# sadPororo/AD-YOLO

Hardware: AMD Instinct MI355X
Metric: train-step audio-sec/s (4ch, se-resnet34+adyolo) (higher is better)
Workload: dtype f32; 1 GPU; se-resnet34 + adyolo loss, synthetic 4ch 24kHz 60s clips, bs=64 per GPU, 12 classes, features+fwd+loss+bwd+allreduce+Adam; global_batch=64, parallelism=dp1

## Files before the change

### ad-yolo_amd/_lib.py

```python
import ctypes
import os

_HERE = os.path.dirname(os.path.abspath(__file__))
LIB_PATH = os.environ.get("ADYOLO_LIB") or os.path.join(_HERE, "libadyolo_hip.so")

P = ctypes.c_void_p
I = ctypes.c_int
L = ctypes.c_long
F = ctypes.c_float
U64 = ctypes.c_uint64

SIGNATURES = {
    "adyolo_abi_version": (I, []),
    "adyolo_last_error": (ctypes.c_char_p, []),
    "adyolo_feat_stft_mel": (I, [P] * 8 + [I, I] + [P] * 4 + [I, I, I, P]),
    "adyolo_feat_finish": (I, [P] * 4 + [I, I, I, P]),
    "adyolo_feat_gcc_phat": (I, [P] * 6 + [I, I, I, I, P]),
    "adyolo_nchw_to_nhwc8": (I, [P, P, I, I, I, I, P]),
    "adyolo_pack_w3x3": (I, [P, P, P, I, I, I, P]),
    "adyolo_conv3x3_tiles": (I, [I] * 3),
    "adyolo_conv3x3_fwd": (I, [P] * 13 + [I] * 7 + [P]),
    "adyolo_wino_pack_w": (I, [P, P, P, I, I, I, P]),
    "adyolo_wino_pack_many": (I, [P, I, I, I, P]),
    "adyolo_wino_tiles": (I, [I] * 3),
    "adyolo_wino_fwd": (I, [P] * 13 + [I] * 7 + [P]),
    "adyolo_wino4_pack_w": (I, [P, P, P, I, I, I, P]),
    "adyolo_wino4_pack_many": (I, [P, I, I, I, P]),
    "adyolo_wino4_tiles": (I, [I] * 3),
    "adyolo_wino4_fwd": (I, [P] * 13 + [I] * 7 + [P]),
    "adyolo_wino4_fwd_form": (I, [I] * 3),
    "adyolo_wino4_last_form": (I, []),
    "adyolo_set_switches": (I, [I]),
    "adyolo_wino4_wgrad_slabs": (I, [I] * 5),
    "adyolo_wino4_wgrad": (I, [P] * 7 + [I] * 6 + [P]),
    "adyolo_wino_wgrad_slabs": (I, [I] * 5),
    "adyolo_wino_wgrad": (I, [P] * 7 + [I] * 6 + [P]),
    "adyolo_conv3x3_wgrad_slabs": (I, [I] * 5),
    "adyolo_conv3x3_wgrad": (I, [P] * 6 + [I] * 6 + [P]),
    "adyolo_gemm": (I, [P] * 5 + [I] * 10 + [P]),
    "adyolo_gemm_batched": (I, [P] * 3 + [I] * 10 + [L] * 6 + [F, I, P]),
    "adyolo_colsum": (I, [P, P, P, I, I, I, I, P]),
    "adyolo_bn_stats": (I, [P] * 7 + [I, I, I, F, F, P]),
    "adyolo_bn_stats_tiles": (I, [P] * 11 + [I, I, I, I, F, F, P]),
    "adyolo_bn_eval_stats": (I, [P] * 4 + [I, F, P]),
    "adyolo_bn_scale_shift": (I, [P] * 6 + [I, P]),
    "adyolo_affine_nhwc": (I, [P] * 4 + [L, I, P]),
    "adyolo_bn_bwd_reduce": (I, [P] * 7 + [L, I, P]),
    "adyolo_bn_bwd_tiles": (I, [P, P, P, P, I, I, P]),
    "adyolo_bn_bwd_apply": (I, [P] * 12 + [L, I, I, F, P]),
    "adyolo_bn_persample": (I, [P, P, P, I, I, I, P]),
    "adyolo_bn_finish": (I, [P] * 10 + [I, I, I, F, F, P]),
    "adyolo_se_fc_fwd": (I, [P] * 10 + [I, I, I, I, P]),
    "adyolo_relu_mask_words": (L, [I, I, I]),
    "adyolo_se_tail_fwd": (I, [P] * 9 + [I, I, I, P]),
    "adyolo_se_tail_fwd_pool_ok": (I, [I, I, I]),
    "adyolo_se_tail_fwd_pool": (I, [P] * 9 + [I, I, I, I, P]),
    "adyolo_se_tail_bwd_reduce": (I, [P] * 9 + [I, I, I, P]),
    "adyolo_se_tail_bwd_tiles": (I, [P, P, P, I, I, I, P]),
    "adyolo_se_fc_bwd_words": (L, [I, I]),
    "adyolo_se_fc_bwd": (I, [P] * 16 + [I, I, I, I, P]),
    "adyolo_se_tail_bwd_apply": (I, [P] * 13 + [I, I, I, F, P]),
    "adyolo_se_tail_bwd_reduce_pooled": (I, [P] * 8 + [I, I, I, I, P]),
    "adyolo_se_tail_bwd_apply_pooled": (I, [P] * 13 + [I, I, I, I, F, P]),
    "adyolo_avgpool2_fwd": (I, [P, P, I, I, I, I, P]),
    "adyolo_avgpool2_bwd": (I, [P, P, I, I, I, I, P]),
    "adyolo_add": (I, [P, P, P, L, P]),
    "adyolo_mul": (I, [P, P, P, L, P]),
    "adyolo_scale_dev": (I, [P, P, P, L, P]),
    "adyolo_sap_fwd": (I, [P] * 5 + [I, I, I, P]),
    "adyolo_sap_bwd": (I, [P] * 8 + [I, I, I, P]),
    "adyolo_gru_fwd": (I, [P] * 6 + [I, I, P]),
    "adyolo_gru_bwd": (I, [P] * 6 + [I, I, P]),
# ... 113 lines not shown
```

### ad-yolo_amd/csrc/gemm.hip

```cpp
#include "common.hpp"

namespace adyolo {

constexpr int GBM = 128, GBN = 64, GBK = 32;
#ifndef GEMM_WHATIF
#define GEMM_WHATIF 0
#endif
#ifndef GEMM_ST_NT
#define GEMM_ST_NT 0
#endif
#ifndef GEMM_PF
#define GEMM_PF 1
#endif

struct GemmBatch {
    int inner;
    long oA, iA, oB, iB, oC, iC;
    float alpha;
};

struct ConvGather {
    int Hs, Ws, Cs, Hm, Wm, KH, KW, SH, SW, PH, PW, dgrad, kreal;
};

// ... 386 lines not shown
#pragma unroll
        for (int nt = 0; nt < SN; ++nt) {
            const int nn = n0 + (wn * SN + nt) * 32 + li;
#pragma unroll
            for (int r = 0; r < 16; ++r) {
                const int m = m0 + (wm * SM + sm) * 32 + mfma_row(r, lane);
                if (m < M && nn < N && (!(GEMM_WHATIF & 1) || r == 0)) {
                    if (slab_stride) {
                        C[(size_t)z * slab_stride + (size_t)m * slab_ld + nn] = acc[sm][nt][r];
                    } else {
                        float v = acc[sm][nt][r] * bt.alpha;
                        if (bias) v += bias[nn];
                        const size_t o = (size_t)m * ldc + nn;
                        if (accumulate) v += C[o];
                        C[o] = v;
                    }
                }
            }
        }
}

__global__ void gemm_slab_reduce_kernel(const float *__restrict__ slabs, const float *__restrict__ bias,
                                        float *__restrict__ C, int M, int N, int ldc, int splits, int accumulate) {
    const size_t idx = (size_t)blockIdx.x * blockDim.x + threadIdx.x;
    const size_t total = (size_t)M * N;
    if (idx >= total) return;
    const int m = (int)(idx / N), nn = (int)(idx - (size_t)m * N);
    float s = 0.f;
    for (int z = 0; z < splits; ++z) s += slabs[(size_t)z * total + idx];
    if (bias) s += bias[nn];
    const size_t o = (size_t)m * ldc + nn;
    if (accumulate) s += C[o];
    C[o] = s;
}

__global__ __launch_bounds__(256) void colsum_partial_kernel(const float *__restrict__ A, float *__restrict__ partial,
                                                             long R, int C, int lda, long rows_per_block) {
    __shared__ float red[256];
    const int cx = threadIdx.x & 63, ry = threadIdx.x >> 6;
    const int c = blockIdx.y * 64 + cx;
    const long rbeg = (long)blockIdx.x * rows_per_block;
    const long rend = rbeg + rows_per_block < R ? rbeg + rows_per_block : R;
    float s = 0.f;
    if (c < C)
        for (long r = rbeg + ry; r < rend; r += 4) s += A[(size_t)r * lda + c];
    red[threadIdx.x] = s;
    __syncthreads();
    if (ry == 0 && c < C) partial[(size_t)blockIdx.x * C + c] = red[cx] + red[64 + cx] + red[128 + cx] + red[192 + cx];
}
__global__ __launch_bounds__(256) void colsum_final_kernel(const float *__restrict__ partial, float *__restrict__ out,
                                                           int nblk, int C, int accumulate) {
    __shared__ double red[256];
    const double s = block_colsum32(partial, nblk, (size_t)C, blockIdx.x * 32, C, red);
    const int c = blockIdx.x * 32 + (threadIdx.x & 31);
    if ((threadIdx.x >> 5) == 0 && c < C) out[c] = (accumulate ? out[c] : 0.f) + (float)s;
}

__global__ void add_kernel(const float4 *__restrict__ a, const float4 *__restrict__ b, float4 *__restrict__ y,
                           long n4) {
    for (long i = (long)blockIdx.x * blockDim.x + threadIdx.x; i < n4; i += (long)gridDim.x * blockDim.x) {
        const float4 u = a[i], v = b[i];
        y[i] = make_float4(u.x + v.x, u.y + v.y, u.z + v.z, u.w + v.w);
    }
}
__global__ void mul_kernel(const float4 *__restrict__ a, const float4 *__restrict__ b, float4 *__restrict__ y,
                           long n4) {
// ... 118 lines not shown
    } else if (mode == 1) {
        M = N * H * W, Nn = Cin, K = Kq;
        cg = ConvGather{Ho, Wo, Cout, H, W, KH, KW, SH, SW, PH, PW, 1, KH * KW * Cout};
    } else {
        M = Cout, Nn = Kp, K = N * Ho * Wo;
        cg = ConvGather{H, W, Cin, Ho, Wo, KH, KW, SH, SW, PH, PW, 0, KH * KW * Cin};
    }
    if (mode != 2 || splits < 1) splits = mode == 2 ? (splits < 1 ? 1 : splits) : 1;
    ADYOLO_REQUIRE(splits == 1 || slabs, ADYOLO_EINVAL, "conv_gemm: splits > 1 needs a slab workspace");
    const int klen = cdiv(cdiv(K, splits), GBK) * GBK;
    splits = cdiv(K, klen);
    int fastg = mode == 2 ? (gemm_fast_fetch(M, 4, K, Cout, 4, 1, 1, klen) & 1)
                          : (gemm_fast_fetch(4, Nn, K, 4, mode == 0 ? Kp : Kq, 0, 0, klen) & 2);
    if (fastg && mode != 2 && cg.Cs % GBK == 0 && (mode == 0 || (SH == 1 && SW == 1)) &&
        (long)N * cg.Hs * cg.Ws * cg.Cs + (long)(KH * cg.Ws + KW) * cg.Cs < ((long)1 << 29))
        fastg |= 4;
    dim3 grid((unsigned)cdiv(Nn, GBN), (unsigned)cdiv(M, GBM), (unsigned)splits);
    const size_t slab_stride = splits > 1 ? (size_t)M * Nn : 0;
    float *dst = splits > 1 ? slabs : out;
    if (mode == 2)
        hipLaunchKernelGGL((gemm_kernel<true, true, 2>), grid, dim3(256), 0, st, other, src, bias, dst, M, Nn, K, Cout, 0,
                           Nn, klen, slab_stride, Nn, 0, bt, cg, fastg);
    else
        hipLaunchKernelGGL((gemm_kernel<false, false, 1>), grid, dim3(256), 0, st, src, other, bias, dst, M, Nn, K, 0,
                           mode == 0 ? Kp : Kq, Nn, klen, slab_stride, Nn, 0, bt, cg, fastg);
    int rc = check_launch("conv_gemm");
    if (rc || splits == 1) return rc;
    const size_t total = (size_t)M * Nn;
    hipLaunchKernelGGL(gemm_slab_reduce_kernel, dim3(cdiv((long)total, 256)), dim3(256), 0, st, slabs, bias, out, M, Nn,
                       Nn, splits, 0);
    return check_launch("conv_gemm_reduce");
}

extern "C" int adyolo_colsum(const float *A, float *out, float *partial, int R, int C, int lda, int accumulate,
                             void *stream) {
    ADYOLO_REQUIRE(A && out && partial && R > 0 && C > 0, ADYOLO_EINVAL, "colsum: bad arguments");
    hipStream_t st = as_stream(stream);
    int nblk = cdiv(R, 64);
    if (nblk > 1024) nblk = 1024;
    const long rpb = ((long)R + nblk - 1) / nblk;
    nblk = cdiv(R, rpb);
    hipLaunchKernelGGL(colsum_partial_kernel, dim3(nblk, cdiv(C, 64)), dim3(256), 0, st, A, partial, (long)R, C, lda, rpb);
    int rc = check_launch("colsum_partial");
    if (rc) return rc;
    hipLaunchKernelGGL(colsum_final_kernel, dim3(cdiv(C, 32)), dim3(256), 0, st, partial, out, nblk, C, accumulate);
    return check_launch("colsum_final");
}

extern "C" int adyolo_add(const float *a, const float *b, float *y, long n, void *stream) {
    ADYOLO_REQUIRE(a && b && y && n > 0 && n % 4 == 0, ADYOLO_EINVAL, "add: n must be a positive multiple of 4");
    const long n4 = n / 4;
    const int grid = (int)(n4 / 256 + 1 > 4096 ? 4096 : n4 / 256 + 1);
    hipLaunchKernelGGL(add_kernel, dim3(grid), dim3(256), 0, as_stream(stream), (const float4 *)a, (const float4 *)b,
                       (float4 *)y, n4);
    return check_launch("add");
}
extern "C" int adyolo_mul(const float *a, const float *b, float *y, long n, void *stream) {
    ADYOLO_REQUIRE(a && b && y && n > 0 && n % 4 == 0, ADYOLO_EINVAL, "mul: n must be a positive multiple of 4");
    const long n4 = n / 4;
    const int grid = (int)(n4 / 256 + 1 > 4096 ? 4096 : n4 / 256 + 1);
    hipLaunchKernelGGL(mul_kernel, dim3(grid), dim3(256), 0, as_stream(stream), (const float4 *)a, (const float4 *)b,
                       (float4 *)y, n4);
    return check_launch("mul");
}
```

### ad-yolo_amd/csrc/wino4w.hip

```cpp
#include "wino4_common.hpp"

namespace adyolo {
namespace w4 {

#ifndef W4W_WHATIF
#define W4W_WHATIF 0
#endif
#ifndef W4W_LD_AUX
#define W4W_LD_AUX 0
#endif
#ifndef W4W_TIMING
#define W4W_TIMING 0
#endif

__device__ __forceinline__ void a6v(const f32x4 (&v)[4], f32x4 (&t)[6]) {
    auto fm = [](float k, f32x4 a, f32x4 b) { return pkfma4(k, a, b); };
    const f32x4 z = {0.f, 0.f, 0.f, 0.f};
    const f32x4 ea = fm(A2, v[2], v[0]), oa = fm(A3, v[3], fm(PA, v[1], z));
    const f32x4 eb = fm(B2, v[2], v[0]), ob = fm(B3, v[3], fm(PB, v[1], z));
    t[0] = v[0];
    t[1] = ea + oa;
    t[2] = fm(-1.f, oa, ea);
    t[3] = eb + ob;
    t[4] = fm(-1.f, ob, eb);
// ... 364 lines not shown
            }
            tstamp(2);
            if (NB == 2) {
                d_xform_full();
                __builtin_amdgcn_sched_barrier(0);
#pragma unroll
                for (int s = 0; s < 9; ++s) {
                    side(9 + s);
                    __builtin_amdgcn_sched_barrier(0);
                    mfma4(s, 1);
                    __builtin_amdgcn_sched_barrier(0);
                }
            }
            tstamp(3);
            tstamp(4);
#if W4W_TIMING
            ++tstep;
#endif
        };
        for (int k = 0; k < nsteps;) {
            step(std::integral_constant<int, 0>{}, k);
            if (++k >= nsteps) break;
            step(std::integral_constant<int, 4>{}, k);
            if (++k >= nsteps) break;
            step(std::integral_constant<int, 8>{}, k);
            if (++k >= nsteps) break;
            step(std::integral_constant<int, 2>{}, k);
            if (++k >= nsteps) break;
            step(std::integral_constant<int, 6>{}, k);
            ++k;
        }
    }

#pragma unroll
    for (int s = 0; s < 9; ++s) {
        const int pos = wave * 9 + s;
#pragma unroll
        for (int cb = 0; cb < NB; ++cb)
#pragma unroll
            for (int r = 0; r < 16; ++r) {
                const int m = mfma_row(r, lane);
                slabs[(((size_t)split * 36 + pos) * Cin + c0 + m) * Cout + co0 + cb * 32 + li] = acc[s][cb][r];
            }
    }
}

__global__ __launch_bounds__(256) void wino4_wgrad_reduce_kernel(const float *__restrict__ slabs, float *__restrict__ du, int nslab,
                                                                 int pairs) {
    __shared__ double red[256];
    const int p = blockIdx.y, total = 36 * pairs;
    const double s = block_colsum32(slabs, nslab, (size_t)total, p * pairs + blockIdx.x * 32, p * pairs + pairs, red);
    const int idx = blockIdx.x * 32 + (threadIdx.x & 31);
    if ((threadIdx.x >> 5) == 0 && idx < pairs) du[(size_t)p * pairs + idx] = (float)s;
}
__global__ __launch_bounds__(256) void wino4_wgrad_finish_kernel(const float *__restrict__ du, float *__restrict__ dw, int Cin,
                                                                 int Cin_real, int Cout) {
    const int pairs = Cin * Cout;
    const int idx = blockIdx.x * blockDim.x + threadIdx.x;
    if (idx >= pairs) return;
    const int co = idx % Cout, ci = idx / Cout;
    if (ci >= Cin_real) return;
    double d[6][6];
#pragma unroll
    for (int wv = 0; wv < 4; ++wv)
#pragma unroll
        for (int s = 0; s < 9; ++s) {
            const int p = wv * 9 + s;
            const int nu = s < 6 ? (wv == 0 ? 0 : wv == 1 ? 2 : wv == 2 ? 3 : 5) : (wv < 2 ? 1 : 4);
            const int xi = s < 6 ? s : (wv & 1) ? (s == 6 ? 5 : s - 4) : s - 6;
            d[xi][nu] = (double)du[(size_t)p * pairs + idx];
        }
    const double a_ = 0.75, b_ = 1.5, a2 = a_ * a_, b2 = b_ * b_;
    const double na = 2.0 * a2 * (a2 - b2), nb = 2.0 * b2 * (b2 - a2);
    const double G[6][3] = {{1.0 / (a2 * b2), 0.0, 0.0}, {1.0 / na, a_ / na, a2 / na}, {1.0 / na, -a_ / na, a2 / na},
                            {1.0 / nb, b_ / nb, b2 / nb}, {1.0 / nb, -b_ / nb, b2 / nb}, {0.0, 0.0, 1.0}};
    float *o = dw + ((size_t)co * Cin_real + ci) * 9;
#pragma unroll
    for (int ky = 0; ky < 3; ++ky)
#pragma unroll
        for (int kx = 0; kx < 3; ++kx) {
            double s_ = 0.0;
#pragma unroll
            for (int xi = 0; xi < 6; ++xi) {
                double r_ = 0.0;
#pragma unroll
                for (int nu = 0; nu < 6; ++nu) r_ += d[xi][nu] * G[nu][kx];
                s_ += G[xi][ky] * r_;
            }
            o[ky * 3 + kx] = (float)s_;
        }
}

static int wino4_wgrad_geometry(int N, int H, int W, int Cin, int Cout, int *npairs_o, int *nseg_o, int *seg_steps_o, int *nitems_o,
                                int *nblk_o) {
    const int nruns = W >= 16 ? N * (W / 16) : cdiv(N, 16 / W), npairs = (nruns + 1) / 2;
    const int nblk = (Cout / (Cout % 64 == 0 ? 64 : 32)) * (Cin / 32);
    int nsplit = 256 / nblk;
    if (nsplit < 1) nsplit = 1;
    const int steps = H / 4;
    int nseg = 1, seg_steps = steps;
    {
        long best = -1;
        const int maxseg = steps >= 16 ? steps / 8 : 1;
        for (int c = 1; c <= maxseg; ++c) {
            const int ss = (steps + c - 1) / c;
            const int ns = (steps + ss - 1) / ss;
            const long items = (long)npairs * ns;
            const int sp = nsplit < items ? nsplit : (int)items;
            const long cost = ((items + sp - 1) / sp) * (long)(ss + 2);
            if (best < 0 || cost < best) {
                best = cost;
                nseg = ns;
                seg_steps = ss;
            }
        }
    }
    const int nitems = npairs * nseg;
    if (nsplit > nitems) nsplit = nitems;
    if (npairs_o) *npairs_o = npairs;
    if (nseg_o) *nseg_o = nseg;
    if (seg_steps_o) *seg_steps_o = seg_steps;
    if (nitems_o) *nitems_o = nitems;
    if (nblk_o) *nblk_o = nblk;
    return nsplit;
}

}
}

using namespace adyolo;

#if W4W_TIMING
extern "C" int adyolo_w4w_timing_buffer(void *p) {
    return hipMemcpyToSymbol(HIP_SYMBOL(w4::g_w4w_stamps), &p, sizeof(p)) == hipSuccess ? 0 : -1;
}
#endif

extern "C" int adyolo_wino4_wgrad_slabs(int N, int H, int W, int Cin, int Cout) {
    if (N <= 0 || H <= 0 || W <= 0 || Cin <= 0 || Cout <= 0) return ADYOLO_EINVAL;
    if (Cin % 32 || Cout % 32 || (W % 16 && W != 4 && W != 8) || H % 4 || H < 8) return 0;
    if ((size_t)N * H * W * (size_t)(Cin > Cout ? Cin : Cout) * 4 >= ((size_t)1 << 31)) return 0;
    return w4::wino4_wgrad_geometry(N, H, W, Cin, Cout, nullptr, nullptr, nullptr, nullptr, nullptr);
}

extern "C" int adyolo_wino4_wgrad(const float *x, const float *dy, const float *in_scale, const float *in_shift, float *slabs,
                                  float *du, float *dw, int N, int H, int W, int Cin, int Cin_real, int Cout, void *stream) {
    ADYOLO_REQUIRE(x && dy && slabs && du && dw && N > 0 && H > 0 && W > 0, ADYOLO_EINVAL, "wino4_wgrad: bad arguments");
    ADYOLO_REQUIRE(adyolo_wino4_wgrad_slabs(N, H, W, Cin, Cout) > 0 && Cin_real > 0 && Cin_real <= Cin, ADYOLO_ENOSUP,
                   "wino4_wgrad: unsupported shape N=%d H=%d W=%d Cin=%d Cout=%d (needs Cin %% 32 == 0, Cout %% 32 == 0, W %% 16 == 0 or W = 4 | 8, "
                   "H %% 4 == 0, tensors below 2 GiB)", N, H, W, Cin, Cout);
    ADYOLO_REQUIRE((in_scale == nullptr) == (in_shift == nullptr), ADYOLO_EINVAL, "wino4_wgrad: in_scale/in_shift come together");
    ADYOLO_REQUIRE(((reinterpret_cast<size_t>(x) | reinterpret_cast<size_t>(dy) | reinterpret_cast<size_t>(in_scale) |
                     reinterpret_cast<size_t>(in_shift)) & 15) == 0, ADYOLO_ENOSUP, "wino4_wgrad: x, dy, in_scale, in_shift must be 16-byte aligned");
    hipStream_t st = as_stream(stream);
    int npairs, nseg, seg_steps, nitems, nblk;
    const int nsplit = w4::wino4_wgrad_geometry(N, H, W, Cin, Cout, &npairs, &nseg, &seg_steps, &nitems, &nblk);
    const unsigned grid = (unsigned)(nsplit * nblk);
#define ADYOLO_W4W(AFF_, NB_)                                                                                          \
    hipLaunchKernelGGL((w4::wino4_wgrad_kernel<AFF_, NB_>), dim3(grid), dim3(256), 0, st, x, dy, in_scale, in_shift, slabs, N, H, \
                       W, Cin, Cout, W >= 16 ? W / 16 : -(W / 4), npairs, nseg, seg_steps, nitems, nsplit, Cin / 32, nblk)
    if (Cout % 64 == 0) {
        if (in_scale) ADYOLO_W4W(true, 2); else ADYOLO_W4W(false, 2);
    } else {
        if (in_scale) ADYOLO_W4W(true, 1); else ADYOLO_W4W(false, 1);
    }
#undef ADYOLO_W4W
    int rc = check_launch("wino4_wgrad");
    if (rc) return rc;
    hipLaunchKernelGGL(w4::wino4_wgrad_reduce_kernel, dim3(cdiv(Cin * Cout, 32), 36), dim3(256), 0, st, slabs, du, nsplit, Cin * Cout);
    rc = check_launch("wino4_wgrad_reduce");
    if (rc) return rc;
    hipLaunchKernelGGL(w4::wino4_wgrad_finish_kernel, dim3(cdiv(Cin * Cout, 256)), dim3(256), 0, st, du, dw, Cin, Cin_real, Cout);
    return check_launch("wino4_wgrad_finish");
}
```

### ad-yolo_amd/ops.py

```python
import ctypes
import os

import numpy as np
import torch

from . import _lib

_c = _lib.call
NULL = ctypes.c_void_p(0)


def _p(t):
    if t is None:
        return NULL
    return ctypes.c_void_p(t.data_ptr())


def _stream():
    return ctypes.c_void_p(torch.cuda.current_stream().cuda_stream)


def _chk(*ts):
    for t in ts:
        if t is None:
# ... 265 lines not shown
    if isinstance(wpk, DualPack):
        wpk = wpk.pick(n, h, w, cout, addend is not None, w4_form == 2)
    form = wpk.shape[0] if wpk.dim() == 4 else 0
    if form == 36 and not w4_form:
        raise _lib.AdyoloHipError("conv3x3: a F(4x4) pack with %d output channels needs an operand combination the persistent kernel "
                                  "is built for (pack with ops.DualPack / WinoPackSet to fall back to F(2x2))" % cout)
    fn, tiles_fn, name = _CONV3X3_FORMS[form]
    _chk(x, wpk, bias, addend, None if mbits & 1 else addend_mask, None if mbits & 2 else stat_mask)
    y = _new(x, n, h, w, cout)
    stats = _new(x, 2, getattr(lib, tiles_fn)(n, h, w), cout) if want_stats else None
    sc, sh = in_affine if in_affine is not None else (None, None)
    sa, sm, si = stat_bn if stat_bn is not None else (None, None, None)
    _c(fn, _p(x), _p(wpk), _p(bias), _p(addend), _p(addend_mask),
       _p(sc), _p(sh), _p(y), _p(stats), _p(sa), _p(sm), _p(si), _p(stat_mask), n, h, w, cin, cout, int(relu), mbits,
       _stream())
    if DISPATCH_LOG is not None:
        k = (name or _W4_KERNELS[w4_form], cin, cout, epi)
        DISPATCH_LOG[k] = DISPATCH_LOG.get(k, 0) + 1
    return (y, stats) if want_stats else y


def wgrad_form(cin, cout, algo=None, shape=None):
    algo = algo or W4_THRESHOLDS["wgrad_algo"] or conv_algo()
    if algo == "winograd4" and shape is not None and cin % 32 == 0 and cout % 32 == 0:
        n, h, w = shape
        if (w % 16 == 0 or w in (4, 8)) and h % 4 == 0 and n * w // 16 * (h // 4) * cin * cout >= W4_THRESHOLDS["min_wgrad_work"] and \
                _lib.load().adyolo_wino4_wgrad_slabs(n, h, w, cin, cout) > 0:
            return "wino4_wgrad_kernel", 9.0 / 36.0
    if algo in ("winograd", "winograd4") and cin % 32 == 0 and cout % 32 == 0:
        return "wino_wgrad_kernel", 16.0 / 36.0
    return "conv3x3_wgrad_kernel", 1.0


_WGRAD_FORMS = {"wino4_wgrad_kernel": ("adyolo_wino4_wgrad", 36), "wino_wgrad_kernel": ("adyolo_wino_wgrad", 16)}


def conv3x3_wgrad(x, dy, cin_real, in_affine=None, algo=None, out=None):
    _chk(x, dy)
    n, h, w, cin = x.shape
    cout = dy.shape[3]
    sc, sh = in_affine if in_affine is not None else (None, None)
    dw = out if out is not None else _new(x, cout, cin_real, 3, 3)
    form = wgrad_form(cin, cout, algo, (n, h, w))[0]
    if DISPATCH_LOG is not None:
        k = (form, cin, cout, 1 if in_affine is not None else 0)
        DISPATCH_LOG[k] = DISPATCH_LOG.get(k, 0) + 1
    if form in _WGRAD_FORMS:
        fn, points = _WGRAD_FORMS[form]
        nslab = getattr(_lib.load(), fn + "_slabs")(n, h, w, cin, cout)
        if nslab <= 0:
            raise _lib.AdyoloHipError("%s_slabs rejected the shape" % fn)
        slabs = _new(x, nslab, points, cin, cout)
        du = _new(x, points, cin, cout)
        _c(fn, _p(x), _p(dy), _p(sc), _p(sh), _p(slabs), _p(du), _p(dw), n, h, w, cin, cin_real, cout, _stream())
        return dw
    nslab = _lib.load().adyolo_conv3x3_wgrad_slabs(n, h, w, cin, cout)
    if nslab <= 0:
        raise _lib.AdyoloHipError("conv3x3_wgrad_slabs rejected the shape")
    cinp = ((cin + 31) // 32) * 32
    slabs = _new(x, nslab, cout, 9, cinp)
    _c("adyolo_conv3x3_wgrad", _p(x), _p(dy), _p(sc), _p(sh), _p(slabs), _p(dw), n, h, w, cin, cin_real, cout, _stream())
    return dw


def gemm(a, b, m, n, k, lda, ldb, trans_a=False, trans_b=False, bias=None, out=None, ldc=None, accumulate=False,
         splits=1):
    if ldc is None:
        ldc = n
    if out is None:
        out = _new(a, m, n)
        ldc = n
    slabs = None
    if splits > 1:
        slabs = _new(a, splits, m, n)
    _c("adyolo_gemm", _p(a), _p(b), _p(bias), _p(out), _p(slabs), m, n, k, lda, ldb, ldc, int(trans_a), int(trans_b),
       splits, int(accumulate), _stream())
    return out


def wgrad_splits(m, n, k):
    tiles = ((m + 127) // 128) * ((n + 63) // 64)
    want = (512 + tiles - 1) // tiles
    return max(1, min(256, want, k // 512))


def linear(x2d, w, bias=None):
    _chk(x2d, w, bias)
    r, k = x2d.shape
    return gemm(x2d, w, r, w.shape[0], k, k, k, bias=bias)


def linear_bwd(x2d, w, dy2d, need_dx=True, out_dw=None, out_db=None, need_db=True):
    _chk(x2d, w, dy2d)
    r, k = x2d.shape
    n = w.shape[0]
    dx = gemm(dy2d, w, r, k, n, n, k, trans_b=True) if need_dx else None
    dw = gemm(dy2d, x2d, n, k, r, n, k, trans_a=True, trans_b=True, splits=wgrad_splits(n, k, r), out=out_dw)
    db = colsum(dy2d, out=out_db) if need_db else None
    return dx, dw, db


def colsum(a2d, out=None, accumulate=False):
    r, c = a2d.shape
    if out is None:
        out = _new(a2d, c)
        accumulate = False
    partial = _new(a2d, 1024, c)
    _c("adyolo_colsum", _p(a2d), _p(out), _p(partial), r, c, a2d.stride(0), int(accumulate), _stream())
    return out


def add(a, b):
    _chk(a, b)
    y = torch.empty_like(a)
    _c("adyolo_add", _p(a), _p(b), _p(y), a.numel(), _stream())
    return y


def scale_dev(a, scalar_dev):
    _chk(a, scalar_dev)
    y = torch.empty_like(a)
    _c("adyolo_scale_dev", _p(a), _p(scalar_dev), _p(y), a.numel(), _stream())
    return y


def mul(a, b):
    _chk(a, b)
    y = torch.empty_like(a)
    _c("adyolo_mul", _p(a), _p(b), _p(y), a.numel(), _stream())
# ... 975 lines not shown
```

### include/adyolo_hip.h

```cpp
#ifndef ADYOLO_HIP_H
#define ADYOLO_HIP_H

#include <stddef.h>
#include <stdint.h>

#ifdef __cplusplus
extern "C" {
#endif

#define ADYOLO_ABI_VERSION 2
#define ADYOLO_EINVAL (-1)
#define ADYOLO_ENOSUP (-2)

int         adyolo_abi_version(void);
const char *adyolo_last_error(void);

int adyolo_feat_stft_mel(const float *audio, const int64_t *clip_offset, const float *twiddle,
                         const int32_t *chunk_mel, const int32_t *chunk_start, const int32_t *chunk_len,
                         const int32_t *chunk_off, const float *mel_w, int n_chunks, int n_mel_w,
                         const float *scaler_mean, const float *scaler_rstd, float *out, float *chan_max, int B,
                         int n_samples, int layout, void *stream);
int adyolo_feat_finish(float *out, const float *chan_max, const float *scaler_mean,
                       const float *scaler_rstd, int B, int T, int layout, void *stream);

// ... 7 lines not shown
                     void *stream);
int adyolo_conv3x3_tiles(int N, int H, int W);
int adyolo_conv3x3_fwd(const float *x, const float *wpk, const float *bias, const float *addend,
                       const float *addend_mask, const float *in_scale, const float *in_shift, float *y,
                       float *stats, const float *stat_aux, const float *stat_mean, const float *stat_invstd,
                       const float *stat_mask, int N, int H, int W, int Cin, int Cout, int relu, int mask_bits, void *stream);
int adyolo_wino_pack_w(const float *w , float *u_fwd , float *u_dgrad ,
                       int Cout, int Cin_real, int Cin, void *stream);
int adyolo_wino_pack_many(const int64_t *table, int n, int max_cout, int max_cin, void *stream);
int adyolo_wino_tiles(int N, int H, int W);
int adyolo_wino_fwd(const float *x, const float *u, const float *bias, const float *addend,
                    const float *addend_mask, const float *in_scale, const float *in_shift, float *y, float *stats,
                    const float *stat_aux, const float *stat_mean, const float *stat_invstd, const float *stat_mask,
                    int N, int H, int W, int Cin, int Cout, int relu, int mask_bits, void *stream);
int adyolo_wino4_pack_w(const float *w , float *u_fwd , float *u_dgrad ,
                        int Cout, int Cin_real, int Cin, void *stream);
int adyolo_wino4_pack_many(const int64_t *table, int n, int max_cout, int max_cin, void *stream);
int adyolo_wino4_tiles(int N, int H, int W);
int adyolo_wino4_fwd(const float *x, const float *u, const float *bias, const float *addend, const float *addend_mask,
                     const float *in_scale, const float *in_shift, float *y, float *stats, const float *stat_aux,
                     const float *stat_mean, const float *stat_invstd, const float *stat_mask, int N, int H, int W, int Cin,
                     int Cout, int relu, int mask_bits, void *stream);
#define ADYOLO_W4_STATS 1
#define ADYOLO_W4_ADDEND 2
#define ADYOLO_W4_ADDEND_MASK 4
#define ADYOLO_W4_STAT_AUX 8
#define ADYOLO_W4_STAT_MASK 16
#define ADYOLO_W4_BIAS 32
int adyolo_wino4_fwd_form(int Cout, int operands, int mask_bits);
int adyolo_wino4_last_form(void);
int adyolo_set_switches(int bits);
int adyolo_wino4_wgrad_slabs(int N, int H, int W, int Cin, int Cout);
int adyolo_wino4_wgrad(const float *x, const float *dy, const float *in_scale , const float *in_shift ,
                       float *slabs, float *du , float *dw, int N, int H, int W, int Cin, int Cin_real,
                       int Cout, void *stream);
int adyolo_wino_wgrad_slabs(int N, int H, int W, int Cin, int Cout);
int adyolo_wino_wgrad(const float *x, const float *dy, const float *in_scale, const float *in_shift, float *slabs,
                      float *du, float *dw, int N, int H, int W, int Cin, int Cin_real, int Cout, void *stream);
int adyolo_conv3x3_wgrad_slabs(int N, int H, int W, int Cin, int Cout);
int adyolo_conv3x3_wgrad(const float *x, const float *dy, const float *in_scale, const float *in_shift,
                         float *slabs, float *dw, int N, int H, int W, int Cin, int Cin_real, int Cout,
                         void *stream);

int adyolo_gemm(const float *A, const float *B, const float *bias, float *C, float *slabs, int M,
                int N, int K, int lda, int ldb, int ldc, int transA, int transB, int splits,
                int accumulate, void *stream);
int adyolo_gemm_batched(const float *A, const float *B, float *C, int M, int N, int K, int lda, int ldb, int ldc,
                        int transA, int transB, int outer, int inner, long oA, long iA, long oB, long iB, long oC,
                        long iC, float alpha, int accumulate, void *stream);
int adyolo_colsum(const float *A, float *out, float *partial, int R, int C, int lda, int accumulate,
                  void *stream);

int adyolo_bn_stats(const float *x, float *ssum, float *mean, float *invstd, float *running_mean,
                    float *running_var, float *partial, int N, int HW, int C, float momentum,
                    float eps, void *stream);
int adyolo_bn_stats_tiles(const float *tile_stats, float *ssum, float *mean, float *invstd, float *running_mean,
                          float *running_var, const float *gamma, const float *beta, float *scale, float *shift,
                          float *partial, int N, int G, int HW, int C, float momentum, float eps, void *stream);
int adyolo_bn_persample(const float *tile_stats, float *ps0, float *ps1, int N, int G, int C, void *stream);
int adyolo_bn_finish(const float *ps0, const float *ps1, float *mean, float *invstd, float *running_mean,
                     float *running_var, const float *gamma, const float *beta, float *scale, float *shift, int N,
                     int HW, int C, float momentum, float eps, void *stream);
int adyolo_bn_eval_stats(const float *running_mean, const float *running_var, float *mean,
                         float *invstd, int C, float eps, void *stream);
int adyolo_bn_scale_shift(const float *gamma, const float *beta, const float *mean,
                          const float *invstd, float *scale, float *shift, int C, void *stream);
int adyolo_affine_nhwc(const float *x, const float *scale, const float *shift, float *y, long rows,
                       int C, void *stream);
int adyolo_bn_bwd_reduce(const float *dy, const float *x, const float *mean, const float *invstd,
                         float *sdy, float *sdyx, float *partial, long rows, int C, void *stream);
int adyolo_bn_bwd_tiles(const float *tile_stats, float *sdy, float *sdyx, float *partial , int tiles, int C,
                        void *stream);
int adyolo_bn_bwd_apply(const float *dy, const float *x, const float *gamma, const float *mean,
                        const float *invstd, const float *sdy, const float *sdyx, float *dx,
                        float *dgamma, float *dbeta, float *dx_colsum ,
                        float *colsum_partial , long rows, int C, int relu_mask,
                        float count_scale ,
                        void *stream);

// ... 208 lines not shown
```

Baseline: 36700 audio-s/s.

## Add streaming TN GEMM for weight grads and fold Winograd wgrad transform into kernel

Adds a streaming split-K TN GEMM kernel that spreads a long K dimension across CUs with MFMA, reduces inside LDS, and computes the bias column sum in the same pass. It is used for large-K weight-gradient GEMMs and linear backward. Separately, the Winograd F(4,3) weight-gradient kernel now applies the output filter transform in-kernel before writing slabs. This cuts slabs from 36 to 9 points and removes the separate finish kernel and du buffer. The cost is more complex epilogues, extra LDS traffic and synchronisation, and a changed transform precision path.

```diff
diff --git a/ad-yolo_amd/_lib.py b/ad-yolo_amd/_lib.py
--- a/ad-yolo_amd/_lib.py
+++ b/ad-yolo_amd/_lib.py
@@ -32,12 +32,14 @@
     "adyolo_wino4_last_form": (I, []),
     "adyolo_set_switches": (I, [I]),
     "adyolo_wino4_wgrad_slabs": (I, [I] * 5),
-    "adyolo_wino4_wgrad": (I, [P] * 7 + [I] * 6 + [P]),
+    "adyolo_wino4_wgrad": (I, [P] * 6 + [I] * 6 + [P]),
     "adyolo_wino_wgrad_slabs": (I, [I] * 5),
     "adyolo_wino_wgrad": (I, [P] * 7 + [I] * 6 + [P]),
     "adyolo_conv3x3_wgrad_slabs": (I, [I] * 5),
     "adyolo_conv3x3_wgrad": (I, [P] * 6 + [I] * 6 + [P]),
     "adyolo_gemm": (I, [P] * 5 + [I] * 10 + [P]),
+    "adyolo_gemm_tn_stream_parts": (I, [I, I, L, I, I]),
+    "adyolo_gemm_tn_stream": (I, [P] * 5 + [I, I, L, I, I, I, I, P]),
     "adyolo_gemm_batched": (I, [P] * 3 + [I] * 10 + [L] * 6 + [F, I, P]),
     "adyolo_colsum": (I, [P, P, P, I, I, I, I, P]),
     "adyolo_bn_stats": (I, [P] * 7 + [I, I, I, F, F, P]),
diff --git a/ad-yolo_amd/csrc/gemm.hip b/ad-yolo_amd/csrc/gemm.hip
--- a/ad-yolo_amd/csrc/gemm.hip
+++ b/ad-yolo_amd/csrc/gemm.hip
@@ -442,6 +442,158 @@
     const size_t o = (size_t)m * ldc + nn;
     if (accumulate) s += C[o];
     C[o] = s;
+}
+
+constexpr int TNS_WAVES = 8;
+template <int T>
+__device__ __forceinline__ void tns_load(__amdgpu_buffer_rsrc_t rs, unsigned off, float (&v)[T]) {
+    if constexpr (T == 4) {
+        const f32x4 t = __builtin_bit_cast(f32x4, __builtin_amdgcn_raw_buffer_load_b128(rs, (int)off, 0, 0));
+        v[0] = t.x; v[1] = t.y; v[2] = t.z; v[3] = t.w;
+    } else if constexpr (T == 2) {
+        const float2 t = __builtin_bit_cast(float2, __builtin_amdgcn_raw_buffer_load_b64(rs, (int)off, 0, 0));
+        v[0] = t.x; v[1] = t.y;
+    } else {
+        v[0] = __builtin_bit_cast(float, __builtin_amdgcn_raw_buffer_load_b32(rs, (int)off, 0, 0));
+    }
+}
+
+template <int TM, int TN>
+__global__ __launch_bounds__(64 * TNS_WAVES, 1) void gemm_tn_stream_kernel(const float *__restrict__ A, const float *__restrict__ B,
+                                                                           float *__restrict__ parts, int M, int N, long K, int lda,
+                                                                           int ldb, long chunk, int MB, int NB, int KW,
+                                                                           int want_colsum) {
+    constexpr int U = 24 / (TM + TN);
+    constexpr int TILE = TM * TN * 1024;
+    extern __shared__ __attribute__((aligned(16))) float tns_lds[];
+    __shared__ float cs_lds[TNS_WAVES][32 * TM];
+    const int lane = threadIdx.x & 63, wave = threadIdx.x >> 6, li = lane & 31, lh = lane >> 5;
+    const int WB = MB * NB;
+    const int wb = wave % WB, kw = wave / WB;
+    const int mb = wb % MB, nb = wb / MB;
+    const int m0 = mb * 32 * TM, n0 = nb * 32 * TN;
+    const long rbeg = ((long)blockIdx.x * KW + kw) * chunk;
+    const long rend = rbeg + chunk < K ? rbeg + chunk : K;
+
+    f32x16 acc[TM][TN];
+    float cs[TM];
+#pragma unroll
+    for (int a = 0; a < TM; ++a) {
+        cs[a] = 0.f;
+#pragma unroll
+        for (int b = 0; b < TN; ++b)
+#pragma unroll
+            for (int r = 0; r < 16; ++r) acc[a][b][r] = 0.f;
+    }
+    if (kw < KW && rbeg < rend) {
+        const int nrows = (int)(rend - rbeg);
+        const __amdgpu_buffer_rsrc_t rsA = __builtin_amdgcn_make_buffer_rsrc(const_cast<float *>(A + rbeg * lda), 0,
+                                                                             ((nrows - 1) * lda + M) * 4, 0x00020000);
+        const __amdgpu_buffer_rsrc_t rsB = __builtin_amdgcn_make_buffer_rsrc(const_cast<float *>(B + rbeg * ldb), 0,
+                                                                             ((nrows - 1) * ldb + N) * 4, 0x00020000);
+        const int colA = m0 + li * TM, colB = n0 + li * TN;
+        const unsigned voA = colA < M ? (unsigned)(lh * lda + colA) * 4u : 0x80000000u;
+        const unsigned voB = colB < N ? (unsigned)(lh * ldb + colB) * 4u : 0x80000000u;
+        const unsigned pairA = (unsigned)lda * 8u, pairB = (unsigned)ldb * 8u;
+        const int nit = (nrows + 2 * U - 1) / (2 * U);
+        float a0[U][TM], b0[U][TN], a1[U][TM], b1[U][TN];
+        auto load = [&](float (&av)[U][TM], float (&bv)[U][TN], int it) {
+#pragma unroll
+            for (int u = 0; u < U; ++u) {
+                tns_load<TM>(rsA, voA + (unsigned)(it * U + u) * pairA, av[u]);
+                tns_load<TN>(rsB, voB + (unsigned)(it * U + u) * pairB, bv[u]);
+            }
+        };
+        auto compute = [&](const float (&av)[U][TM], const float (&bv)[U][TN]) {
+#pragma unroll
+            for (int u = 0; u < U; ++u)
+#pragma unroll
+                for (int a = 0; a < TM; ++a) {
+                    cs[a] += av[u][a];
+#pragma unroll
+                    for (int b = 0; b < TN; ++b) acc[a][b] = mfma32(av[u][a], bv[u][b], acc[a][b]);
+                }
+        };
+        load(a0, b0, 0);
+        for (int it = 0; it < nit; it += 2) {
+            load(a1, b1, it + 1);
+            compute(a0, b0);
+            load(a0, b0, it + 2);
+            compute(a1, b1);
+        }
+    }
+    for (int h = KW >> 1; h >= 1; h >>= 1) {
+        if (kw >= h && kw < 2 * h) {
+            float *img = tns_lds + (size_t)((kw - h) * WB + wb) * TILE;
+#pragma unroll
+            for (int a = 0; a < TM; ++a)
+#pragma unroll
+                for (int b = 0; b < TN; ++b)
+#pragma unroll
+                    for (int r = 0; r < 16; ++r) img[((a * TN + b) * 16 + r) * 64 + lane] = acc[a][b][r];
+        }
+        __syncthreads();
+        if (kw < h) {
+            const float *img = tns_lds + (size_t)(kw * WB + wb) * TILE;
+#pragma unroll
+            for (int a = 0; a < TM; ++a)
+#pragma unroll
+                for (int b = 0; b < TN; ++b)
+#pragma unroll
+                    for (int r = 0; r < 16; ++r) acc[a][b][r] += img[((a * TN + b) * 16 + r) * 64 + lane];
+        }
+        __syncthreads();
+    }
+    float *part = parts + (size_t)blockIdx.x * ((size_t)M * N + M);
+    if (want_colsum) {
+        if (kw < KW && nb == 0) {
+#pragma unroll
+            for (int a = 0; a < TM; ++a) {
+                const float t = cs[a] + __shfl_xor(cs[a], 32, 64);
+                if (lh == 0) cs_lds[wave][li * TM + a] = t;
+            }
+        }
+        __syncthreads();
+        if (kw == 0 && nb == 0 && lh == 0) {
+#pragma unroll
+            for (int a = 0; a < TM; ++a) {
+                float t = 0.f;
+                for (int q = 0; q < KW; ++q) t += cs_lds[q * WB + wb][li * TM + a];
+                const int m = m0 + li * TM + a;
+                if (m < M) part[(size_t)M * N + m] = t;
+            }
+        }
+    }
+    if (kw == 0) {
+#pragma unroll
+        for (int a = 0; a < TM; ++a)
+#pragma unroll
+            for (int r = 0; r < 16; ++r) {
+                const int m = m0 + mfma_row(r, lane) * TM + a;
+                const int nn = n0 + li * TN;
+                if (m < M && nn < N) {
+                    if constexpr (TN == 2) *reinterpret_cast<float2 *>(part + (size_t)m * N + nn) = make_float2(acc[a][0][r], acc[a][1][r]);
+                    else part[(size_t)m * N + nn] = acc[a][0][r];
+                }
+            }
+    }
+}
+
+__global__ __launch_bounds__(256) void tn_stream_reduce_kernel(const float *__restrict__ parts, float *__restrict__ C,
+                                                               float *__restrict__ colsum_out, int nparts, int M, int N, int ldc,
+                                                               int accumulate) {
+    __shared__ double red[256];
+    const int total = M * N + (colsum_out ? M : 0);
+    const double s = block_colsum32(parts, nparts, (size_t)M * N + M, blockIdx.x * 32, total, red);
+    const int e = blockIdx.x * 32 + (threadIdx.x & 31);
+    if ((threadIdx.x >> 5) != 0 || e >= total) return;
+    if (e >= M * N) {
+        colsum_out[e - M * N] = (float)s;
+    } else {
+        const int m = e / N;
+        const size_t o = (size_t)m * ldc + (e - m * N);
+        C[o] = (accumulate ? C[o] : 0.f) + (float)s;
+    }
 }
 
 __global__ __launch_bounds__(256) void colsum_partial_kernel(const float *__restrict__ A, float *__restrict__ partial,
@@ -626,6 +778,73 @@
     return check_launch("conv_gemm_reduce");
 }
 
+struct TnsPlan {
+    int tm, tn, mb, nb, kw, nwg;
+    long chunk;
+};
+static TnsPlan tns_plan(int M, int N, long K, int lda, int ldb) {
+    TnsPlan p{0, 0, 0, 0, 0, 0, 0};
+    if (M <= 0 || N <= 0 || K <= 0 || M > 256 || N > 256 || (M & 3) || (N & 3) || (lda & 3) || (ldb & 3) || lda < M || ldb < N) return p;
+    static int cus = 0;
+    if (cus == 0) {
+        int dev = 0, v = 0;
+        if (hipGetDevice(&dev) != hipSuccess || hipDeviceGetAttribute(&v, hipDeviceAttributeMultiprocessorCount, dev) != hipSuccess || v < 1)
+            return p;
+        cus = v > 256 ? 256 : v;
+    }
+    const int m32 = cdiv(M, 32), n32 = cdiv(N, 32);
+    p.tm = m32 >= 3 ? 4 : m32;
+    p.tn = n32 >= 2 ? 2 : 1;
+    p.mb = cdiv(m32, p.tm);
+    p.nb = cdiv(n32, p.tn);
+    p.kw = TNS_WAVES / (p.mb * p.nb);
+    long chunk = (K + (long)cus * p.kw - 1) / ((long)cus * p.kw);
+    chunk = (chunk + 1) & ~1L;
+    if (chunk < 16) chunk = 16;
+    p.chunk = chunk;
+    p.nwg = cdiv(K, chunk * p.kw);
+    if (chunk * (lda > ldb ? lda : ldb) >= ((long)1 << 28)) p.nwg = 0;
+    return p;
+}
+
+extern "C" int adyolo_gemm_tn_stream_parts(int M, int N, long K, int lda, int ldb) { return tns_plan(M, N, K, lda, ldb).nwg; }
+
+extern "C" int adyolo_gemm_tn_stream(const float *A, const float *B, float *C, float *colsum_out, float *parts, int M, int N,
+                                     long K, int lda, int ldb, int ldc, int accumulate, void *stream) {
+    ADYOLO_REQUIRE(A && B && C && parts, ADYOLO_EINVAL, "gemm_tn_stream: bad arguments");
+    const TnsPlan p = tns_plan(M, N, K, lda, ldb);
+    ADYOLO_REQUIRE(p.nwg > 0 && ldc >= N, ADYOLO_ENOSUP,
+                   "gemm_tn_stream: M=%d N=%d K=%ld lda=%d ldb=%d ldc=%d is not a shape of the streaming form", M, N, K, lda, ldb, ldc);
+    hipStream_t st = as_stream(stream);
+    const int want_cs = colsum_out != nullptr;
+#define LAUNCH_TNS(TM_, TN_)                                                                                                  \
+    do {                                                                                                                      \
+        const size_t lds = (size_t)(TNS_WAVES / 2) * TM_ * TN_ * 1024 * sizeof(float);                                        \
+        static bool attr_set = false;                                                                                         \
+        if (!attr_set && lds > 48 * 1024) {                                                                                   \
+            const hipError_t e = hipFuncSetAttribute(reinterpret_cast<const void *>(&gemm_tn_stream_kernel<TM_, TN_>),         \
+                                                     hipFuncAttributeMaxDynamicSharedMemorySize, (int)lds);                   \
+            ADYOLO_REQUIRE(e == hipSuccess, (int)e, "gemm_tn_stream: %s", hipGetErrorString(e));                              \
+            attr_set = true;                                                                                                  \
+        }                                                                                                                     \
+        hipLaunchKernelGGL((gemm_tn_stream_kernel<TM_, TN_>), dim3(p.nwg), dim3(64 * TNS_WAVES), lds, st, A, B, parts, M, N, K, \
+                           lda, ldb, p.chunk, p.mb, p.nb, p.kw, want_cs);                                                     \
+    } while (0)
+    if (p.tm == 4 && p.tn == 2) LAUNCH_TNS(4, 2);
+    else if (p.tm == 4) LAUNCH_TNS(4, 1);
+    else if (p.tm == 2 && p.tn == 2) LAUNCH_TNS(2, 2);
+    else if (p.tm == 2) LAUNCH_TNS(2, 1);
+    else if (p.tn == 2) LAUNCH_TNS(1, 2);
+    else LAUNCH_TNS(1, 1);
+#undef LAUNCH_TNS
+    int rc = check_launch("gemm_tn_stream");
+    if (rc) return rc;
+    const int total = M * N + (want_cs ? M : 0);
+    hipLaunchKernelGGL(tn_stream_reduce_kernel, dim3(cdiv(total, 32)), dim3(256), 0, st, parts, C, colsum_out, p.nwg, M, N, ldc,
+                       accumulate);
+    return check_launch("gemm_tn_stream_reduce");
+}
+
 extern "C" int adyolo_colsum(const float *A, float *out, float *partial, int R, int C, int lda, int accumulate,
                              void *stream) {
     ADYOLO_REQUIRE(A && out && partial && R > 0 && C > 0, ADYOLO_EINVAL, "colsum: bad arguments");
diff --git a/ad-yolo_amd/csrc/wino4w.hip b/ad-yolo_amd/csrc/wino4w.hip
--- a/ad-yolo_amd/csrc/wino4w.hip
+++ b/ad-yolo_amd/csrc/wino4w.hip
@@ -420,63 +420,62 @@
         }
     }
 
-#pragma unroll
-    for (int s = 0; s < 9; ++s) {
-        const int pos = wave * 9 + s;
-#pragma unroll
-        for (int cb = 0; cb < NB; ++cb)
+    {
+        constexpr double a_ = 0.75, b_ = 1.5, a2 = a_ * a_, b2 = b_ * b_;
+        constexpr double na = 2.0 * a2 * (a2 - b2), nb = 2.0 * b2 * (b2 - a2);
+        constexpr double G0 = 1.0 / (a2 * b2), Ga0 = 1.0 / na, Ga1 = a_ / na, Ga2 = a2 / na, Gb0 = 1.0 / nb, Gb1 = b_ / nb, Gb2 = b2 / nb;
+        auto gt = [&](double v0, double v1, double v2, double v3, double v4, double v5, double &o0, double &o1, double &o2) {
+            const double sa = v1 + v2, da = v1 - v2, sb = v3 + v4, db = v3 - v4;
+            o0 = G0 * v0 + Ga0 * sa + Gb0 * sb;
+            o1 = Ga1 * da + Gb1 * db;
+            o2 = Ga2 * sa + Gb2 * sb + v5;
+        };
+        float *xch = lds;
+        __syncthreads();
+#pragma unroll
+        for (int cb = 0; cb < NB; ++cb) {
 #pragma unroll
             for (int r = 0; r < 16; ++r) {
-                const int m = mfma_row(r, lane);
-                slabs[(((size_t)split * 36 + pos) * Cin + c0 + m) * Cout + co0 + cb * 32 + li] = acc[s][cb][r];
-            }
+                double t0, t1, t2, p0, p1, p2;
+                gt(acc[0][cb][r], acc[1][cb][r], acc[2][cb][r], acc[3][cb][r], acc[4][cb][r], acc[5][cb][r], t0, t1, t2);
+                if (hh == 0) gt(acc[6][cb][r], acc[7][cb][r], acc[8][cb][r], 0.0, 0.0, 0.0, p0, p1, p2);
+                else gt(0.0, 0.0, 0.0, acc[7][cb][r], acc[8][cb][r], acc[6][cb][r], p0, p1, p2);
+                float *o = xch + ((wave * 6) * 16 + r) * 64 + lane;
+                o[0 * 1024] = (float)t0; o[1 * 1024] = (float)t1; o[2 * 1024] = (float)t2;
+                o[3 * 1024] = (float)p0; o[4 * 1024] = (float)p1; o[5 * 1024] = (float)p2;
+            }
+            __syncthreads();
+#pragma unroll
+            for (int rr = 0; rr < 4; ++rr) {
+                const int r = wave * 4 + rr;
+                const float *in = xch + r * 64 + lane;
+                float *o = slabs + (((size_t)split * 9) * Cin + c0 + mfma_row(r, lane)) * Cout + co0 + cb * 32 + li;
+#pragma unroll
+                for (int ky = 0; ky < 3; ++ky) {
+                    const double v0 = in[(0 * 6 + ky) * 1024], v2 = in[(1 * 6 + ky) * 1024], v3 = in[(2 * 6 + ky) * 1024], v5 = in[(3 * 6 + ky) * 1024];
+                    const double v1 = (double)in[(0 * 6 + 3 + ky) * 1024] + (double)in[(1 * 6 + 3 + ky) * 1024];
+                    const double v4 = (double)in[(2 * 6 + 3 + ky) * 1024] + (double)in[(3 * 6 + 3 + ky) * 1024];
+                    double w0, w1, w2;
+                    gt(v0, v1, v2, v3, v4, v5, w0, w1, w2);
+                    o[(size_t)(ky * 3 + 0) * Cin * Cout] = (float)w0;
+                    o[(size_t)(ky * 3 + 1) * Cin * Cout] = (float)w1;
+                    o[(size_t)(ky * 3 + 2) * Cin * Cout] = (float)w2;
+                }
+            }
+            if (cb + 1 < NB) __syncthreads();
+        }
     }
 }
 
-__global__ __launch_bounds__(256) void wino4_wgrad_reduce_kernel(const float *__restrict__ slabs, float *__restrict__ du, int nslab,
-                                                                 int pairs) {
+__global__ __launch_bounds__(256) void wino4_wgrad_reduce_kernel(const float *__restrict__ slabs, float *__restrict__ dw, int nslab,
+                                                                 int Cin, int Cin_real, int Cout) {
     __shared__ double red[256];
-    const int p = blockIdx.y, total = 36 * pairs;
-    const double s = block_colsum32(slabs, nslab, (size_t)total, p * pairs + blockIdx.x * 32, p * pairs + pairs, red);
+    const int pairs = Cin * Cout, tap = blockIdx.y, total = 9 * pairs;
+    const double s = block_colsum32(slabs, nslab, (size_t)total, tap * pairs + blockIdx.x * 32, tap * pairs + pairs, red);
     const int idx = blockIdx.x * 32 + (threadIdx.x & 31);
-    if ((threadIdx.x >> 5) == 0 && idx < pairs) du[(size_t)p * pairs + idx] = (float)s;
-}
-__global__ __launch_bounds__(256) void wino4_wgrad_finish_kernel(const float *__restrict__ du, float *__restrict__ dw, int Cin,
-                                                                 int Cin_real, int Cout) {
-    const int pairs = Cin * Cout;
-    const int idx = blockIdx.x * blockDim.x + threadIdx.x;
-    if (idx >= pairs) return;
+    if ((threadIdx.x >> 5) != 0 || idx >= pairs) return;
     const int co = idx % Cout, ci = idx / Cout;
-    if (ci >= Cin_real) return;
-    double d[6][6];
-#pragma unroll
-    for (int wv = 0; wv < 4; ++wv)
-#pragma unroll
-        for (int s = 0; s < 9; ++s) {
-            const int p = wv * 9 + s;
-            const int nu = s < 6 ? (wv == 0 ? 0 : wv == 1 ? 2 : wv == 2 ? 3 : 5) : (wv < 2 ? 1 : 4);
-            const int xi = s < 6 ? s : (wv & 1) ? (s == 6 ? 5 : s - 4) : s - 6;
-            d[xi][nu] = (double)du[(size_t)p * pairs + idx];
-        }
-    const double a_ = 0.75, b_ = 1.5, a2 = a_ * a_, b2 = b_ * b_;
-    const double na = 2.0 * a2 * (a2 - b2), nb = 2.0 * b2 * (b2 - a2);
-    const double G[6][3] = {{1.0 / (a2 * b2), 0.0, 0.0}, {1.0 / na, a_ / na, a2 / na}, {1.0 / na, -a_ / na, a2 / na},
-                            {1.0 / nb, b_ / nb, b2 / nb}, {1.0 / nb, -b_ / nb, b2 / nb}, {0.0, 0.0, 1.0}};
-    float *o = dw + ((size_t)co * Cin_real + ci) * 9;
-#pragma unroll
-    for (int ky = 0; ky < 3; ++ky)
-#pragma unroll
-        for (int kx = 0; kx < 3; ++kx) {
-            double s_ = 0.0;
-#pragma unroll
-            for (int xi = 0; xi < 6; ++xi) {
-                double r_ = 0.0;
-#pragma unroll
-                for (int nu = 0; nu < 6; ++nu) r_ += d[xi][nu] * G[nu][kx];
-                s_ += G[xi][ky] * r_;
-            }
-            o[ky * 3 + kx] = (float)s_;
-        }
+    if (ci < Cin_real) dw[((size_t)co * Cin_real + ci) * 9 + tap] = (float)s;
 }
 
 static int wino4_wgrad_geometry(int N, int H, int W, int Cin, int Cout, int *npairs_o, int *nseg_o, int *seg_steps_o, int *nitems_o,
@@ -532,8 +531,8 @@
 }
 
 extern "C" int adyolo_wino4_wgrad(const float *x, const float *dy, const float *in_scale, const float *in_shift, float *slabs,
-                                  float *du, float *dw, int N, int H, int W, int Cin, int Cin_real, int Cout, void *stream) {
-    ADYOLO_REQUIRE(x && dy && slabs && du && dw && N > 0 && H > 0 && W > 0, ADYOLO_EINVAL, "wino4_wgrad: bad arguments");
+                                  float *dw, int N, int H, int W, int Cin, int Cin_real, int Cout, void *stream) {
+    ADYOLO_REQUIRE(x && dy && slabs && dw && N > 0 && H > 0 && W > 0, ADYOLO_EINVAL, "wino4_wgrad: bad arguments");
     ADYOLO_REQUIRE(adyolo_wino4_wgrad_slabs(N, H, W, Cin, Cout) > 0 && Cin_real > 0 && Cin_real <= Cin, ADYOLO_ENOSUP,
                    "wino4_wgrad: unsupported shape N=%d H=%d W=%d Cin=%d Cout=%d (needs Cin %% 32 == 0, Cout %% 32 == 0, W %% 16 == 0 or W = 4 | 8, "
                    "H %% 4 == 0, tensors below 2 GiB)", N, H, W, Cin, Cout);
@@ -555,9 +554,7 @@
 #undef ADYOLO_W4W
     int rc = check_launch("wino4_wgrad");
     if (rc) return rc;
-    hipLaunchKernelGGL(w4::wino4_wgrad_reduce_kernel, dim3(cdiv(Cin * Cout, 32), 36), dim3(256), 0, st, slabs, du, nsplit, Cin * Cout);
-    rc = check_launch("wino4_wgrad_reduce");
-    if (rc) return rc;
-    hipLaunchKernelGGL(w4::wino4_wgrad_finish_kernel, dim3(cdiv(Cin * Cout, 256)), dim3(256), 0, st, du, dw, Cin, Cin_real, Cout);
-    return check_launch("wino4_wgrad_finish");
-}
+    hipLaunchKernelGGL(w4::wino4_wgrad_reduce_kernel, dim3(cdiv(Cin * Cout, 32), 9), dim3(256), 0, st, slabs, dw, nsplit, Cin, Cin_real,
+                       Cout);
+    return check_launch("wino4_wgrad_reduce");
+}
diff --git a/ad-yolo_amd/ops.py b/ad-yolo_amd/ops.py
--- a/ad-yolo_amd/ops.py
+++ b/ad-yolo_amd/ops.py
@@ -321,7 +321,7 @@
     return "conv3x3_wgrad_kernel", 1.0
 
 
-_WGRAD_FORMS = {"wino4_wgrad_kernel": ("adyolo_wino4_wgrad", 36), "wino_wgrad_kernel": ("adyolo_wino_wgrad", 16)}
+_WGRAD_FORMS = {"wino4_wgrad_kernel": ("adyolo_wino4_wgrad", 9), "wino_wgrad_kernel": ("adyolo_wino_wgrad", 16)}
 
 
 def conv3x3_wgrad(x, dy, cin_real, in_affine=None, algo=None, out=None):
@@ -340,6 +340,9 @@
         if nslab <= 0:
             raise _lib.AdyoloHipError("%s_slabs rejected the shape" % fn)
         slabs = _new(x, nslab, points, cin, cout)
+        if points == 9:
+            _c(fn, _p(x), _p(dy), _p(sc), _p(sh), _p(slabs), _p(dw), n, h, w, cin, cin_real, cout, _stream())
+            return dw
         du = _new(x, points, cin, cout)
         _c(fn, _p(x), _p(dy), _p(sc), _p(sh), _p(slabs), _p(du), _p(dw), n, h, w, cin, cin_real, cout, _stream())
         return dw
@@ -359,6 +362,8 @@
     if out is None:
         out = _new(a, m, n)
         ldc = n
+    if trans_a and trans_b and bias is None and splits > 1 and tn_stream_parts(m, n, k, lda, ldb):
+        return gemm_tn_stream(a, b, m, n, k, lda, ldb, out=out, ldc=ldc, accumulate=accumulate)
     slabs = None
     if splits > 1:
         slabs = _new(a, splits, m, n)
@@ -373,6 +378,28 @@
     return max(1, min(256, want, k // 512))
 
 
+TN_STREAM_MIN_ROWS = int(os.environ.get("ADYOLO_TN_STREAM_MIN_ROWS", "131072"))
+
+
+def tn_stream_parts(m, n, k, lda, ldb):
+    if m > 256 or n > 256 or k < TN_STREAM_MIN_ROWS:
+        return 0
+    return _lib.load().adyolo_gemm_tn_stream_parts(m, n, k, lda, ldb)
+
+
+def gemm_tn_stream(a, b, m, n, k, lda, ldb, out=None, ldc=None, accumulate=False, colsum_out=None):
+    parts = _lib.load().adyolo_gemm_tn_stream_parts(m, n, k, lda, ldb)
+    if parts <= 0:
+        raise _lib.AdyoloHipError("gemm_tn_stream_parts rejected the shape")
+    if out is None:
+        out, ldc, accumulate = _new(a, m, n), n, False
+    elif ldc is None:
+        ldc = n
+    ws = _new(a, parts, m * n + m)
+    _c("adyolo_gemm_tn_stream", _p(a), _p(b), _p(out), _p(colsum_out), _p(ws), m, n, k, lda, ldb, ldc, int(accumulate), _stream())
+    return out
+
+
 def linear(x2d, w, bias=None):
     _chk(x2d, w, bias)
     r, k = x2d.shape
@@ -384,6 +411,10 @@
     r, k = x2d.shape
     n = w.shape[0]
     dx = gemm(dy2d, w, r, k, n, n, k, trans_b=True) if need_dx else None
+    if need_db and wgrad_splits(n, k, r) > 1 and tn_stream_parts(n, k, r, n, k):
+        db = out_db if out_db is not None else _new(dy2d, n)
+        dw = gemm_tn_stream(dy2d, x2d, n, k, r, n, k, out=out_dw, colsum_out=db)
+        return dx, dw, db
     dw = gemm(dy2d, x2d, n, k, r, n, k, trans_a=True, trans_b=True, splits=wgrad_splits(n, k, r), out=out_dw)
     db = colsum(dy2d, out=out_db) if need_db else None
     return dx, dw, db
diff --git a/include/adyolo_hip.h b/include/adyolo_hip.h
--- a/include/adyolo_hip.h
+++ b/include/adyolo_hip.h
@@ -63,8 +63,7 @@
 int adyolo_set_switches(int bits);
 int adyolo_wino4_wgrad_slabs(int N, int H, int W, int Cin, int Cout);
 int adyolo_wino4_wgrad(const float *x, const float *dy, const float *in_scale , const float *in_shift ,
-                       float *slabs, float *du , float *dw, int N, int H, int W, int Cin, int Cin_real,
-                       int Cout, void *stream);
+                       float *slabs, float *dw, int N, int H, int W, int Cin, int Cin_real, int Cout, void *stream);
 int adyolo_wino_wgrad_slabs(int N, int H, int W, int Cin, int Cout);
 int adyolo_wino_wgrad(const float *x, const float *dy, const float *in_scale, const float *in_shift, float *slabs,
                       float *du, float *dw, int N, int H, int W, int Cin, int Cin_real, int Cout, void *stream);
@@ -76,6 +75,9 @@
 int adyolo_gemm(const float *A, const float *B, const float *bias, float *C, float *slabs, int M,
                 int N, int K, int lda, int ldb, int ldc, int transA, int transB, int splits,
                 int accumulate, void *stream);
+int adyolo_gemm_tn_stream_parts(int M, int N, long K, int lda, int ldb);
+int adyolo_gemm_tn_stream(const float *A, const float *B, float *C, float *colsum_out, float *parts, int M, int N,
+                          long K, int lda, int ldb, int ldc, int accumulate, void *stream);
 int adyolo_gemm_batched(const float *A, const float *B, float *C, int M, int N, int K, int lda, int ldb, int ldc,
                         int transA, int transB, int outer, int inner, long oA, long iA, long oB, long iB, long oC,
                         long iC, float alpha, int accumulate, void *stream);
```

Result: no change. 36970 audio-s/s (median of 6 runs) (+0.8%).
